# alshai/Big-BWT

Hardware: AMD Instinct MI355X
Metric: input MB/s to .bwt (bit-exact vs ref) (higher is better)
Workload: dtype u8; 1 GPU; BASELINE configs[2]: 64x mutated yeast-shaped FASTA (~0.79 GB), -w 10 -p 100, BWT + -s -e sampled SA; bytes_per_gpu=787308470, w=10, p=100, flags=6, phrases=16409159, words=921010, dict_bytes=79900101, parallelism=1 GPU

## Files before the change

### big-bwt_amd/csrc/api_stages.hip

```cpp
#include "chain.hpp"

using namespace pfp;

namespace pfp {

__global__ void sorted_len1_kernel(uint32_t d, const uint32_t *__restrict__ word_at_rank,
                                   const uint32_t *__restrict__ wlen, uint32_t *__restrict__ len1) {
  uint32_t r = BID * blockDim.x + threadIdx.x;
  if (r == 0) len1[d] = 0;
  if (r < d) len1[r] = wlen[word_at_rank[r]] + 1;
}

template <class A, class B>
__global__ void convert_kernel(const A *__restrict__ in, uint64_t n, B *__restrict__ out) {
  uint64_t i = (uint64_t)BID * blockDim.x + threadIdx.x;
  if (i < n) out[i] = (B)in[i];
}
template <class A, class B>
static void fetch_converted(pfp_ctx *c, const A *d_in, uint64_t n, B *h_out) {
  if constexpr (sizeof(A) == sizeof(B)) {
    d2h(c, (A *)h_out, d_in, n);
    sync(c);
  } else {
    DBuf<B> tmp(c, n);
// ... 308 lines not shown
              pfp_bwt_result *out) {
  if (!c || !dict || !occ || !ilist || !bwlast || !out) return PFP_EINVAL;
  memset(out, 0, sizeof *out);
  PFP_TRY_DEV(c)
  check_args(w, 10, flags);
  PFP_REQUIRE(!flags || bwsai, PFP_EINVAL, "SA output requested but no bwsai given");
  PFP_REQUIRE(dict_size > 1 + (uint64_t)w, PFP_EFORMAT, "invalid dictionary file (pfbwt.cpp:332)");
  PFP_REQUIRE(ilist[0] == 1, PFP_EFORMAT, "ilist[0] != 1 (pfbwt.cpp:377)");
  PFP_REQUIRE(dict[0] == kDollar, PFP_EFORMAT, "dictionary must start with Dollar (pfbwt.cpp:125)");
  Dictionary D; DictIndex ix; DictOrder ord;
  dictionary_from_host(c, dict, dict_size, D, ix);
  PFP_REQUIRE(D.d == n_words, PFP_EFORMAT, "occ entries != dictionary words (pfbwt.cpp:357)");
  uint64_t expect = 0, tot_occ = 0;
  {
    uint64_t s = 0, j = 0;
    for (uint64_t i = 0; i < dict_size; i++)
      if (dict[i] == kEndOfWord) {
        uint64_t len = i - s;
        if (len > (uint64_t)w) expect += (len - (uint64_t)w) * occ[j];
        tot_occ += occ[j];
        j++; s = i + 1;
      }
  }
  PFP_REQUIRE(tot_occ + 1 == n_plus_1, PFP_EFORMAT, "sum(occ)+1 != parse size (pfbwt.cpp:397)");
  D.wocc.alloc(c, D.d);
  h2d(c, D.wocc.p, occ, D.d);
  if (c->debug) validate_index(c, D, ix);
  const WordView wv = word_view(D, ix);
  const SlotPayloadSrc pay{wv, D.wocc.p, w};
  ord.wide = use_wide_index(c, D.dsize);
  with_width(ord.wide, [&](auto tag) {
    using I = decltype(tag);
    auto &so = ord.get<I>();
    sort_dict_suffixes<I>(c, D.bytes.p, D.dsize, wv, so, (flags & PFP_FLAG_SA) ? nullptr : &pay);
    if (c->debug) validate_suffix_order<I>(c, D.bytes.p, so, true, "dict SA");
    compute_lexrank<I>(c, D, so, ix);
  });
  if (c->debug) validate_lexrank(c, D, ix);
  DBuf<uint32_t> occ_lex(c, D.d);
  occ_in_lex_order(c, (uint32_t)D.d, ix.lexrank.p, D.wocc.p, occ_lex.p, nullptr);
  ParseBWT pb;
  pb.P = n_plus_1 - 1;
  pb.ilist.alloc(c, n_plus_1); pb.bwlast.alloc(c, n_plus_1);
  h2d(c, pb.ilist.p, ilist, n_plus_1); h2d(c, pb.bwlast.p, bwlast, n_plus_1);
  if (flags) {
    DBuf<uint8_t> packed(c, n_plus_1 * 5);
    h2d(c, packed.p, bwsai, n_plus_1 * 5);
    pb.bwsai.alloc(c, n_plus_1);
    unpack5_dev(c, packed.p, n_plus_1, pb.bwsai.p);
// ... 19 lines not shown
```

### big-bwt_amd/csrc/chain.hip

```cpp
#include "chain.hpp"

using namespace pfp;

namespace pfp {

__global__ void occ_lex_kernel(uint32_t d, const uint32_t *__restrict__ lexrank, const uint32_t *__restrict__ wocc,
                               uint32_t *__restrict__ occ_lex, uint32_t *__restrict__ word_at_rank) {
  uint32_t j = BID * blockDim.x + threadIdx.x;
  if (j >= d) return;
  uint32_t r = lexrank[j];
  occ_lex[r] = wocc[j];
  if (word_at_rank) word_at_rank[r] = j;
}
__global__ void parse_sym_kernel(uint64_t P, const uint32_t *__restrict__ pid, const uint32_t *__restrict__ lexrank,
                                 uint32_t *__restrict__ sym) {
  uint64_t k = (uint64_t)BID * blockDim.x + threadIdx.x;
  if (k < P) sym[k] = lexrank[pid[k]] + 1;
}
__global__ __launch_bounds__(256) void dict_permute_kernel(uint32_t d, const uint32_t *__restrict__ word_at_rank,
                                                           const uint64_t *__restrict__ woff,
                                                           const uint32_t *__restrict__ wlen,
                                                           const uint8_t *__restrict__ src,
                                                           const uint64_t *__restrict__ doff, uint8_t *__restrict__ dst) {
  uint64_t t = (uint64_t)BID * 256 + threadIdx.x;
// ... 34 lines not shown
    if (c->debug) validate_dictionary(c, ch.D, w);
    build_dict_index(c, ch.D, ch.ix);
    if (c->debug) validate_index(c, ch.D, ch.ix);
    ch.tx.buf.release();
    ch.ends.release();
  }
  {
    PhaseTimer t(c, &st.ms_sa_dict);
    const WordView wv = word_view(ch.D, ch.ix);
    const SlotPayloadSrc pay{wv, ch.D.wocc.p, w};
    ch.ord.wide = prefer_wide_index(c, ch.D.dsize);
    with_width(ch.ord.wide, [&](auto tag) {
      using I = decltype(tag);
      auto &so = ch.ord.get<I>();
      so.rep_hint = (double)ch.n_used / (double)std::max<uint64_t>(ch.D.dsize, 1);
      sort_dict_suffixes<I>(c, ch.D.bytes.p, ch.D.dsize, wv, so, dense_sa ? nullptr : &pay);
      if (c->debug) validate_suffix_order<I>(c, ch.D.bytes.p, so, true, "dict SA");
      compute_lexrank<I>(c, ch.D, so, ch.ix);
      if (!c->debug) { so.rank.release(); so.tab.release(); }
    });
    if (c->debug) validate_lexrank(c, ch.D, ch.ix);
    const uint32_t d = (uint32_t)ch.D.d;
    ch.occ_lex.alloc(c, d); ch.word_at_rank.alloc(c, d);
    occ_in_lex_order(c, d, ch.ix.lexrank.p, ch.D.wocc.p, ch.occ_lex.p, ch.word_at_rank.p);
    ch.sym.alloc(c, ch.D.P);
    hipLaunchKernelGGL(parse_sym_kernel, gdim(cdiv(ch.D.P, TB)), gdim(TB), 0, c->stream, ch.D.P, ch.D.pid.p,
                       ch.ix.lexrank.p, ch.sym.p);
    PFP_HIP(hipGetLastError());
  }
  st.n = ch.n_used; st.n_phrases = ch.D.P; st.n_words = ch.D.d; st.dict_size = ch.D.dsize;
  st.sa_rounds_dict = ch.ord.rounds(); st.hash_reseeds = ch.D.reseeds; st.index_bits = ch.ord.wide ? 64 : 32;
// ... 234 lines not shown
```

### big-bwt_amd/csrc/common.hpp

```cpp
#pragma once
#include <hip/hip_runtime.h>
#include <cstdint>
#include <cstdio>
#include <cstring>
#include <stdexcept>
#include <string>
#include <vector>
#include <chrono>
#include <map>
#include <thread>
#include "../../include/pfpgpu.h"

struct K1Scratch; struct DistState;
namespace pfp {
struct StagedText;

constexpr uint8_t kDollar = 2, kEndOfWord = 1, kEndOfDict = 0;
constexpr uint32_t kPrime = 1999999973u;

struct Error : std::runtime_error {
  int code;
  Error(int c, const std::string &m) : std::runtime_error(m), code(c) {}
};

// ... 77 lines not shown
      free_list[bi] = free_list.back(); free_list.pop_back();
      for (auto &b : all) if (b.p == p) { b.file = file; b.line = line; b.req = bytes; break; }
      note_peak();
      return p;
    }
    void *p = nullptr;
    hipError_t e = hipMalloc(&p, bytes);
    driver_allocs++;
    if (e != hipSuccess) {
      (void)hipGetLastError();
      trim();
      trims++;
      e = hipMalloc(&p, bytes);
    }
    if (e != hipSuccess) { *err = e; (void)hipGetLastError(); return nullptr; }
    all.push_back({p, bytes, p, file, line, bytes}); total_bytes += bytes;
    live_bytes += bytes; note_peak();
    return p;
  }
  void put(void *p) {
    for (size_t i = 0; i < all.size(); i++)
      if (all[i].p == p) {
        live_bytes -= all[i].req;
        if (debug) { put_debug(i); return; }
        free_list.push_back(all[i]);
        return;
      }
  }
  void *get_debug(size_t bytes, hipError_t *err, const char *file, int line) {
    void *base = nullptr;
// ... 192 lines not shown
```

### big-bwt_amd/csrc/kernels.hpp

```cpp
#pragma once
#include "common.hpp"
#include "wordview.hpp"

namespace pfp {

struct StagedText {
  static constexpr size_t kFront = 64, kBack = 128;
  DBuf<uint8_t> buf;
  uint64_t n = 0;
  int w = 0;
  const uint8_t *tbase() const { return buf.p + kFront; }
  const uint8_t *tprime() const { return buf.p + kFront - 1; }
  void stage(pfp_ctx *c, const void *src, bool src_on_device, uint64_t n_, int w_);
  void stage_fd(pfp_ctx *c, int fd, uint64_t file_off, uint64_t n_, int w_);
  void restage_tail(pfp_ctx *c, uint64_t new_n, int w_) const;
};

struct KRParams {
  static constexpr uint32_t kMaxExtra = 32;
  uint32_t negpw, pinv, pshift, plimit;
  float fdens = 1.0f;
  uint32_t fthr_nom = 0, fauto = 0;
  uint32_t fast = 0, fseed = 0, fthr = 0;
  uint32_t nextra;
// ... 89 lines not shown
  uint64_t n_refined = 0;
};
using SuffixOrder = SuffixOrderT<uint32_t>;
using SuffixOrder64 = SuffixOrderT<uint64_t>;
struct SlotPayloadSrc { WordView wv; const uint32_t *wocc; int w; };
template <class I>
struct RankViewT {
  const I *rank; const uint64_t *skeys; const I *tab; const uint32_t *lut; const uint8_t *bytes;
  uint64_t N; int kbits, shift; uint32_t T; I finbit; uint64_t keymask;
  const I *wordrank;
};
template <class I> RankViewT<I> rank_view(const SuffixOrderT<I> &so);
template <class I> void gather_ranks(pfp_ctx *c, const SuffixOrderT<I> &so, const uint64_t *d_pos, uint64_t count, I *d_out);
template <class I>
void sort_dict_suffixes(pfp_ctx *c, const uint8_t *bytes, uint64_t N, const WordView &wv, SuffixOrderT<I> &out,
                        const SlotPayloadSrc *pay = nullptr);
template <class I>
void sort_dict_suffixes_range(pfp_ctx *c, const uint8_t *bytes, uint64_t N, const WordView &wv, uint32_t part,
                              uint32_t parts, SuffixOrderT<I> &out, const SlotPayloadSrc *pay = nullptr,
                              const SlotPayloadSrc *count = nullptr);
template <class I>
void gather_slots_range(pfp_ctx *c, const SuffixOrderT<I> &so, const WordView &wv, uint64_t count, uint64_t *d_out);
void sort_int_suffixes_range(pfp_ctx *c, const uint32_t *sym, uint64_t N, uint32_t max_sym, const uint32_t *occ, uint32_t n_sym,
                             uint32_t part, uint32_t parts, SuffixOrder &out);
void sort_int_suffixes(pfp_ctx *c, const uint32_t *sym, uint64_t N, SuffixOrder &out, uint32_t max_sym = 0xFFFFFFFFu,
                       const uint32_t *occ = nullptr, uint32_t n_sym = 0);
template <class I> void sort_byte_suffixes(pfp_ctx *c, const uint8_t *bytes, uint64_t N, SuffixOrderT<I> &out);

struct DictIndex {
  DBuf<uint32_t> blk_word;
  DBuf<uint64_t> wend;
// ... 239 lines not shown
```

### big-bwt_amd/csrc/merge.hip

```cpp
#include "kernels.hpp"
#include "prims.hpp"
#include "devutil.hpp"
#include <algorithm>
#include <cstdlib>

namespace pfp {

static constexpr int TB = 256;
constexpr int kOffTileLog = 11;


template <class I> struct alignas(16) Idx8 { I v[8]; };
template <class I>
__global__ __launch_bounds__(256) void slot_payload_kernel(uint64_t N, const I *__restrict__ sa,
                                                           const uint64_t *__restrict__ skeys,
                                                           const uint8_t *__restrict__ refined, const uint8_t *__restrict__ b,
                                                           WordView wv,
                                                           const uint32_t *__restrict__ wocc, uint32_t d, int w,
                                                           uint32_t *__restrict__ cnt, uint8_t *__restrict__ pc) {
  if ((uint64_t)BID * 2048 >= N) return;
  uint64_t t0 = ((uint64_t)BID * 256 + threadIdx.x) * 8;
  uint32_t c8[8], p8[8];
  const int nk = t0 >= N ? 0 : ((N - t0) >= 8 ? 8 : (int)(N - t0));
  uint64_t rf = 0;
// ... 1375 lines not shown
    sync(c);
    for (uint32_t q = 0; q < nbig; q++) hg.es[q + 1] = hg.es[q] + hb[q].E;
    hg.estart.alloc(c, nbig + 1);
    PFP_HIP(hipMemcpyAsync(hg.estart.p, hg.es.data(), (nbig + 1) * 8, hipMemcpyHostToDevice, c->stream));
    sync(c);
  }

  void queued_groups(int pass) {
    const MergeArgsT<I> ap = with_pass(pass);
    const std::vector<uint64_t> &es = hg.es;
    if (hg.nmid) {
      KScope ks(c, "pfp::hard_sort_kernel", (uint64_t)hg.nmid * (kHardSortMin + 1) * (sa_mode ? 21 : 5));
      hipLaunchKernelGGL(hard_sort_kernel<I>, gdim(c->n_cu * 4), gdim(256), 0, c->stream, ap, hg.mid.p, hg.nmid);
      PFP_HIP(hipGetLastError());
    }
    for (uint32_t q0 = 0; q0 < hg.nbig;) {
      uint32_t q1 = q0 + 1;
      while (q1 < hg.nbig && es[q1 + 1] - es[q0] <= sw.big_budget) q1++;
      const uint64_t cnt = es[q1] - es[q0];
      if (cnt > sw.big_budget) {
        const int nb = (int)std::min<uint64_t>(cdiv64(cnt, 256), (uint64_t)c->n_cu * 32);
        KScope ks(c, "pfp::hard_big_kernel", cnt * (sa_mode ? 21 : 5));
        hipLaunchKernelGGL(hard_big_kernel<I>, gdim(nb), gdim(256), 0, c->stream, ap, hg.big.p + q0, q1 - q0, hg.estart.p + q0, cnt);
      } else {
        DBuf<uint64_t> bk(c, cnt), bka(c, cnt), bv(c, cnt), bva(c, cnt);
        { KScope ks(c, "pfp::big_keys_kernel", cnt * 28);
          hipLaunchKernelGGL(big_keys_kernel<I>, gdim(cdiv(cnt, 256)), gdim(256), 0, c->stream, ap, hg.big.p, q0, q1, hg.estart.p, cnt, bk.p, bv.p); }
        { SortTag tag("large hard groups"); sort_pairs_db<uint64_t, uint64_t>(c, bk, bka, bv, bva, cnt, 0, 32 + bits_for(q1 - q0)); }
        { KScope ks(c, "pfp::big_place_kernel", cnt * (sa_mode ? 34 : 18));
          hipLaunchKernelGGL(big_place_kernel<I>, gdim(cdiv(cnt, 256)), gdim(256), 0, c->stream, ap, hg.big.p, q0, hg.estart.p, cnt, bk.p, bv.p); }
      }
      PFP_HIP(hipGetLastError());
      q0 = q1;
    }
  }

  void mark_run_boundaries() {
    const uint64_t cnt_slice = a.out_hi > a.out_lo ? a.out_hi - a.out_lo : 0;
    const uint64_t nw = cdiv64(cnt_slice, 64);
    out.bmap.alloc(c, nw + 1); out.bpre.alloc(c, nw + 1);
// ... 129 lines not shown
```

### big-bwt_amd/csrc/sufsort.hip

```cpp
#include "kernels.hpp"
#include "prims.hpp"
#include "devutil.hpp"
#include <algorithm>
#include <cmath>
#include <optional>
#include <vector>
#include <cstdio>
#include <cstdlib>

namespace pfp {

enum : int { MODE_DICT = 0, MODE_PLAIN = 1 };

struct SufGeom {
  int mode; uint64_t N; WordView wv;
  const uint32_t *sym = nullptr;
  const uint32_t *dist = nullptr;
};
__device__ __forceinline__ uint64_t suf_len(const SufGeom &g, uint64_t i) {
  if (g.mode == MODE_DICT) return slen_of(g.wv, i) + 1;
  return g.N - i;
}

struct KeyCode {
// ... 113 lines not shown
    if ((L.skeys[mid] & L.keymask) < k) lo = mid + 1; else hi = mid;
  }
  return lo;
}

__device__ __forceinline__ uint32_t slot_record(const uint8_t *__restrict__ b, uint64_t i, uint32_t wd, const SlotPayloadSrc &P) {
  if (!(wd < P.wv.d && P.wv.wend[wd] - i > (uint64_t)P.w)) return 0u;
  const uint32_t pc = (i == 0) ? kEndOfWord : b[i - 1];
  const uint32_t occ = P.wocc[wd];
  return pc | ((occ < 255u ? occ : 255u) << 8);
}
constexpr int kKeyPos = 224;
struct KeyStreamLds { uint32_t off[257]; uint32_t bs[200]; uint32_t wsum[4]; unsigned long long tmask[4]; uint32_t wbase; };
__device__ __forceinline__ uint64_t block_stream_key(KeyStreamLds &L, const uint8_t *__restrict__ s, uint64_t N,
                                                     const KeyCode &kp, uint64_t B0, const WordView *view = nullptr,
                                                     uint32_t *word_out = nullptr) {
  const int t = threadIdx.x, lane = t & 63, wv = t >> 6;
  const uint64_t pos = B0 + t;
  if (t < 200) L.bs[t] = 0;
  const uint32_t c = pos < N ? s[pos] : 0u;
  const uint32_t e = kp.lut[c];
  const uint32_t l = e & 63u, cd = e >> 6;
  uint32_t inc = l;
  for (int o = 1; o < 64; o <<= 1) { const uint32_t v = __shfl_up(inc, o, 64); if (lane >= o) inc += v; }
  if (lane == 63) L.wsum[wv] = inc;
  const unsigned long long tmine = __ballot(c <= (uint32_t)kEndOfWord);
  if (lane == 0) L.tmask[wv] = tmine;
  if (word_out && t == 0) L.wbase = B0 < N ? word_of(*view, B0) : 0u;
  __syncthreads();
  if (word_out) {
    uint32_t before = (uint32_t)__popcll(tmine & ((1ull << lane) - 1ull));
    for (int q = 0; q < wv; q++) before += (uint32_t)__popcll(L.tmask[q]);
    *word_out = L.wbase + before;
  }
  uint32_t base = 0;
  for (int q = 0; q < wv; q++) base += L.wsum[q];
  const uint32_t p = base + inc - l;
  L.off[t] = p;
  if (t == 255) L.off[256] = p + l;
  {
    const uint32_t w = p >> 5, o = p & 31u;
    if (o + l <= 32) atomicOr(&L.bs[w], cd << (32 - o - l));
    else {
      const uint32_t r = o + l - 32;
      atomicOr(&L.bs[w], cd >> r);
      atomicOr(&L.bs[w + 1], (cd & ((1u << r) - 1u)) << (32 - r));
    }
  }
  __syncthreads();
  if (t >= kKeyPos || pos >= N) return 0;
  uint32_t toterm = 33u;
  {
    const unsigned long long m0 = tmine >> lane;
    if (m0) toterm = (uint32_t)__builtin_ctzll(m0) + 1u;
    else if (wv < 3) { const unsigned long long m1 = L.tmask[wv + 1]; if (m1) toterm = (uint32_t)(64 - lane) + (uint32_t)__builtin_ctzll(m1) + 1u; }
    if (toterm > 33u) toterm = 33u;
  }
  const uint32_t nch = toterm < 32u ? toterm : 32u;
  const uint32_t avail = L.off[t + nch] - p;
  const uint32_t kb = (uint32_t)kp.kbits;
  const uint32_t take = avail < kb ? avail : kb;
  const uint32_t w = p >> 5, sh = p & 31u;
  const uint64_t hi = ((uint64_t)L.bs[w] << 32) | L.bs[w + 1];
  uint64_t x = hi << sh;
  if (sh) x |= (uint64_t)(L.bs[w + 2] >> (32 - sh));
  uint64_t k = x >> (64 - kb);
  if (take < kb) k &= ~((1ull << (kb - take)) - 1ull);
  const uint32_t term = (toterm <= 32u && L.off[t + toterm] - p <= kb) ? 1u : 0u;
  return (k << 1) | term;
}
template <class I>
__global__ __launch_bounds__(256) void init_keys_packed_kernel(const uint8_t *__restrict__ s, uint64_t N, KeyCode kp,
                                                               SlotPayloadSrc P, int paybits, uint64_t *__restrict__ key,
                                                               I *__restrict__ val, int idx_bits) {
  __shared__ KeyStreamLds L;
  const uint64_t B0 = (uint64_t)BID * kKeyPos;
  uint32_t wd = 0;
  uint64_t k = paybits ? block_stream_key(L, s, N, kp, B0, &P.wv, &wd) : block_stream_key(L, s, N, kp, B0);
  const uint64_t pos = B0 + threadIdx.x;
  if (threadIdx.x >= kKeyPos || pos >= N) return;
  if (idx_bits) { key[pos] = (k << idx_bits) | pos; return; }
  if (paybits) k |= (uint64_t)slot_record(s, pos, wd, P) << 48;
  key[pos] = k; val[pos] = (I)pos;
}
template <class I>
__global__ void split_keys_kernel(const uint64_t *__restrict__ comb, uint64_t n, int idx_bits, uint64_t *__restrict__ key,
                                  I *__restrict__ val) {
  const uint64_t a = (uint64_t)BID * blockDim.x + threadIdx.x;
  if (a >= n) return;
  const uint64_t x = comb[a];
  key[a] = x >> idx_bits;
  val[a] = (I)(x & ((1ull << idx_bits) - 1ull));
}
__global__ void check_keys_kernel(const uint8_t *__restrict__ s, uint64_t N, KeyCode kp, const uint64_t *__restrict__ key,
                                  uint64_t keymask, unsigned long long *__restrict__ bad, int idx_bits) {
  uint64_t i = (uint64_t)BID * blockDim.x + threadIdx.x;
  if (i >= N) return;
  if (((key[i] >> idx_bits) & keymask) != packed_key_at(s, i, kp.kbits, kp.lut)) atomicAdd(bad, 1ull);
}
template <class I>
__global__ void init_keys_bytes_kernel(const uint8_t *__restrict__ s, uint64_t N, uint64_t *__restrict__ key,
                                       I *__restrict__ val) {
  uint64_t i = (uint64_t)BID * blockDim.x + threadIdx.x;
  if (i >= N) return;
  key[i] = __builtin_bswap64(ld8u(s + i));
  val[i] = (I)i;
}
__global__ void init_keys_int_kernel(const uint32_t *__restrict__ s, uint64_t N, uint64_t *__restrict__ key,
                                     uint32_t *__restrict__ val) {
  uint64_t i = (uint64_t)BID * blockDim.x + threadIdx.x;
  if (i >= N) return;
  uint64_t a = s[i], b = (i + 1 < N) ? s[i + 1] : 0;
  key[i] = (a << 32) | b; val[i] = (uint32_t)i;
// ... 551 lines not shown
  uint32_t pivot_cap = []() { const char *e = getenv("PFP_PIVOT_CAP"); uint32_t v = e ? (uint32_t)atoll(e) : 512u; return v > kPivCapMax ? kPivCapMax : v; }();
};
static const SorterSwitches kSwitch;

template <class I>
RankViewT<I> rank_view(const SuffixOrderT<I> &so) {
  return RankViewT<I>{so.rank.p, so.skeys.p, so.tab.p, so.lut.p, so.bytes, so.N, so.kbits, so.shift, so.T, so.finbit, so.keymask, so.wordrank.p};
}
template RankViewT<uint32_t> rank_view(const SuffixOrderT<uint32_t> &);
template RankViewT<uint64_t> rank_view(const SuffixOrderT<uint64_t> &);

struct DoublingOpts {
  int key_bits = 64;
  bool dict = false;
  std::optional<uint64_t> list_len;
  int idx_bits = 0;
};

enum class Round {
  FirstDict,
  FirstPlain,
  DictPivotGlobal,
  DictPivotGrouped,
  ParsePivot,
  DoublingGlobal,
  DoublingGrouped,
};

template <class I>
struct Rounds {
  using K = typename IdxTraits<I>::DKey;
  static constexpr bool kWide = sizeof(I) == 8;
  static constexpr int TB = 256;

  pfp_ctx *const c;
  const SufGeom g;
  SuffixOrderT<I> &out;
  const DoublingOpts o;
  const uint64_t NP, N;
  const bool lazy;
  const bool range_mode;
  const int nb;
  bool lazy_active = false, late_rank = false;
  I *rank_p = nullptr, *wordrank_p = nullptr;

  Round kind;
  uint64_t m, h, m2 = 0, ngrp = 0;
  uint32_t piv_cap = kSwitch.pivot_cap;
  bool pivot_ok = true;
  bool ipiv_ok = true;
  bool small_failed = false;
  bool finisher_ok = true;
  bool rank_alloc = false;
  bool lazy_pending = false;
  bool ranks_stale = false;
// ... 5 lines not shown
  DBuf<uint64_t> keyo;
  DBuf<I> valo;
  DBuf<uint8_t> hd, keep;
  DBuf<I> aslot, aslot2, hv, newhead, act_i, act_grp;
  uint64_t list_cap = 0;
  DBuf<uint32_t> tile_keep, tile_heads;
  DBuf<I> tile_off, tile_hoff;
  DBuf<uint8_t> keep0, veto;
  DBuf<uint32_t> wstart_bits;
  DBuf<uint8_t> gs, bigf;
  DBuf<uint32_t> k32, k32o, segb, sege, nseg_d, ovf_d;
  DBuf<uint64_t> nsel_d;
  DBuf<K> dkey, dkeyo;

  Rounds(pfp_ctx *c_, const SufGeom &g_, DBuf<uint64_t> &key_, DBuf<I> &val_, uint64_t h0, SuffixOrderT<I> &out_, const DoublingOpts &o_)
      : c(c_), g(g_), out(out_), o(o_), NP(g_.N), N(o_.list_len.value_or(g_.N)), lazy(o_.dict), range_mode(o_.list_len.has_value()),
        nb(bits_for(N)), kind(o_.dict ? Round::FirstDict : Round::FirstPlain), m(N), h(h0), key(key_), val(val_) {}

  static uint64_t blocks(uint64_t n) { return cdiv(n, TB); }

  void first_round_sort() {
    keyo.alloc(c, N); valo.alloc(c, N);
    SortTag first_tag(g.mode == MODE_DICT ? "dictionary, first round" : "parse, first round");
    if (o.idx_bits) {
      if (kSwitch.lib_sort) sort_keys_db(c, key, keyo, N, o.idx_bits, o.idx_bits + o.key_bits);
      else msd_sort_keys_db(c, key, keyo, N, o.idx_bits, o.idx_bits + o.key_bits);
      KScope ks(c, "pfp::split_keys_kernel", N * (16 + sizeof(I)));
      hipLaunchKernelGGL(split_keys_kernel<I>, gdim(blocks(N)), gdim(TB), 0, c->stream, key.p, N, o.idx_bits, keyo.p, valo.p);
    } else {
      if (kSwitch.lib_sort) sort_pairs_db(c, key, keyo, val, valo, N, 0, o.key_bits);
      else msd_sort_pairs_db<I>(c, key, keyo, val, valo, N, 0, o.key_bits);
// ... 359 lines not shown
      if (kind != Round::DoublingGrouped) {
        { KScope ks(c, "pfp::build_keys_kernel", m * (4 + 4 + 4 + 12));
          hipLaunchKernelGGL(build_keys_kernel<I>, gdim(blocks(m)), gdim(TB), 0, c->stream, g, m, h, act_i.p, act_grp.p, L, nb, key.p, val.p); }
        sort_device_wide(keybits);
      }
    }
    h *= 2;
    out.rounds++;
  }

  bool next_round() {
    if (dict_pivot_wanted()) { dict_pivot_round(); return true; }
    if constexpr (!kWide) {
      if (parse_pivot_wanted() && parse_pivot_round()) return true;
    }
    if (range_mode) { out.complete = false; return false; }
    prepare_ranks_for_doubling();
    doubling_round();
    return true;
  }
};

template <class I>
static void doubling(pfp_ctx *c, SufGeom g, DBuf<uint64_t> &key, DBuf<I> &val, uint64_t h0, SuffixOrderT<I> &out, const DoublingOpts &o) {
  Rounds<I> r(c, g, key, val, h0, out, o);
  out.N = r.N; out.NP = r.NP; out.range = r.range_mode; out.complete = true;
  out.rounds = 0;
  if (r.N == 0) { out.sa.alloc(c, 1); out.grp.alloc(c, 8); out.rank.alloc(c, 1); return; }
  r.first_round_sort();
  SortTag later_tag(g.mode == MODE_DICT ? "dictionary, later rounds" : "parse, later rounds");
  r.start_rounds();
// ... 17 lines not shown
    const I r = L.wordrank[a];
    if (r != IdxTraits<I>::kNone) { out[a] = r & ~L.finbit; return; }
  }
  out[a] = rank_at(L, pos[a], settled);
}
template <class I>
void gather_ranks(pfp_ctx *c, const SuffixOrderT<I> &so, const uint64_t *d_pos, uint64_t count, I *d_out) {
  if (!count) return;
  hipLaunchKernelGGL(gather_ranks_kernel<I>, gdim(cdiv(count, 256)), gdim(256), 0, c->stream, rank_view(so), count, d_pos, d_out);
  PFP_HIP(hipGetLastError());
}
template void gather_ranks<uint32_t>(pfp_ctx *, const SuffixOrderT<uint32_t> &, const uint64_t *, uint64_t, uint32_t *);
template void gather_ranks<uint64_t>(pfp_ctx *, const SuffixOrderT<uint64_t> &, const uint64_t *, uint64_t, uint64_t *);


static KeyCode dict_key_code(pfp_ctx *c, const uint8_t *bytes, uint64_t N, double rep_hint = 0) {
  DBuf<unsigned long long> hist(c, 256);
  hist.zero();
  hipLaunchKernelGGL(byte_histogram_kernel, gdim(std::min<uint64_t>(cdiv64(N, 4096), (uint64_t)c->n_cu * 8)), gdim(256), 0,
                     c->stream, bytes, N, hist.p);
  std::vector<uint64_t> hh(256);
  PFP_HIP(hipMemcpyAsync(hh.data(), hist.p, 2048, hipMemcpyDeviceToHost, c->stream));
  sync(c);
  return make_key_code(hh.data(), rep_hint);
}

template <class I>
static int keysonly_bits(uint64_t N, double rep_hint, KeyCode &kc) {
  const int keysonly_env = []() { const char *e = getenv("PFP_KEYSONLY"); return e ? atoi(e) : -1; }();
  if (!(sizeof(I) == 4 && N >= 2 && (keysonly_env == 1 || (keysonly_env != 0 && rep_hint >= 2.0 && N >= (1u << 20))))) return 0;
  const int ib = bits_for(N - 1);
  int width = 64 - ib;
  if (width > 3 * kKeysDigitBits && width % kKeysDigitBits <= 2) width -= width % kKeysDigitBits;
  if (!(width - 1 >= 35 || keysonly_env == 1)) return 0;
  if (kc.kbits > width - 1) { kc.kbits = std::max(8, width - 1); kc.hmin = std::max(1, std::min(32, kc.kbits / kc.maxlen)); }
  return ib;
}

template <class I>
static void require_dict_size(uint64_t N) {
  PFP_REQUIRE(N >= 1 && (sizeof(I) == 8 ? N < (1ull << 40) : N < 0xFFFFFFF0ull), PFP_ELIMIT,
              sizeof(I) == 8 ? "dictionary of 2^40 bytes or more" : "dictionary too large for 32-bit suffix indices");
}
static uint64_t dict_keymask(const KeyCode &kc) { return kc.kbits + 1 >= 64 ? ~0ull : ((1ull << (kc.kbits + 1)) - 1); }

template <class I>
static void dict_rounds(pfp_ctx *c, const SufGeom &g, const uint8_t *bytes, const KeyCode &kc, int idx_bits, std::optional<uint64_t> list_len,
                        DBuf<uint64_t> &key, DBuf<I> &val, SuffixOrderT<I> &out) {
  out.keymask = dict_keymask(kc);
  out.lut.alloc(c, 256);
  PFP_HIP(hipMemcpyAsync(out.lut.p, kc.lut, 1024, hipMemcpyHostToDevice, c->stream));
  sync(c);
  out.bytes = bytes; out.kbits = kc.kbits;
  DoublingOpts o;
  o.key_bits = kc.kbits + 1, o.dict = true, o.list_len = list_len, o.idx_bits = idx_bits;
  doubling<I>(c, g, key, val, (uint64_t)kc.hmin, out, o);
}

template <class I>
void sort_dict_suffixes(pfp_ctx *c, const uint8_t *bytes, uint64_t N, const WordView &wv, SuffixOrderT<I> &out,
                        const SlotPayloadSrc *pay) {
  require_dict_size<I>(N);
  SufGeom g{MODE_DICT, N, wv};
  KeyCode kc = dict_key_code(c, bytes, N, out.rep_hint);
  const int idx_bits = keysonly_bits<I>(N, out.rep_hint, kc);
  DBuf<uint64_t> key(c, N);
  DBuf<I> val;
  if (!idx_bits) val.alloc(c, N);
  out.paybits = (pay && !idx_bits && kc.kbits + 1 <= 48) ? 16 : 0;
  { KScope ks(c, "pfp::init_keys_packed_kernel", N * (9 + (idx_bits ? 0 : sizeof(I)) + (out.paybits ? 9 : 0)));
    hipLaunchKernelGGL(init_keys_packed_kernel<I>, gdim((unsigned)cdiv64(N, kKeyPos)), gdim(256), 0, c->stream, bytes, N, kc,
                       pay ? *pay : SlotPayloadSrc{}, out.paybits, key.p, val.p, idx_bits); }
  if (c->debug) {
    DBuf<unsigned long long> bad(c, 1);
    bad.zero();
    hipLaunchKernelGGL(check_keys_kernel, gdim(cdiv(N, 256)), gdim(256), 0, c->stream, bytes, N, kc, key.p, dict_keymask(kc), bad.p, idx_bits);
    PFP_HIP(hipMemcpyAsync(c->h_scalars, bad.p, 8, hipMemcpyDeviceToHost, c->stream));
    sync(c);
    PFP_REQUIRE(c->h_scalars[0] == 0, PFP_EHIP, "bit-stream keys differ from packed_key_at at " + std::to_string(c->h_scalars[0]) + " positions");
  }
  dict_rounds<I>(c, g, bytes, kc, idx_bits, std::nullopt, key, val, out);
}
template void sort_dict_suffixes<uint32_t>(pfp_ctx *, const uint8_t *, uint64_t, const WordView &, SuffixOrderT<uint32_t> &, const SlotPayloadSrc *);
template void sort_dict_suffixes<uint64_t>(pfp_ctx *, const uint8_t *, uint64_t, const WordView &, SuffixOrderT<uint64_t> &, const SlotPayloadSrc *);


template <class I>
void sort_byte_suffixes(pfp_ctx *c, const uint8_t *bytes, uint64_t N, SuffixOrderT<I> &out) {
  PFP_REQUIRE(N >= 1 && (sizeof(I) == 8 ? N < (1ull << 40) : N < 0xFFFFFFF0ull), PFP_ELIMIT, "text too large for the suffix index width");
  SufGeom g{MODE_PLAIN, N, WordView{}};
  DBuf<uint64_t> key(c, N);
  DBuf<I> val(c, N);
  { KScope ks(c, "pfp::init_keys_bytes_kernel", N * (16 + sizeof(I)));
    hipLaunchKernelGGL(init_keys_bytes_kernel<I>, gdim(cdiv(N, 256)), gdim(256), 0, c->stream, bytes, N, key.p, val.p); }
  doubling<I>(c, g, key, val, 8, out, DoublingOpts{});
}
template void sort_byte_suffixes<uint32_t>(pfp_ctx *, const uint8_t *, uint64_t, SuffixOrderT<uint32_t> &);
template void sort_byte_suffixes<uint64_t>(pfp_ctx *, const uint8_t *, uint64_t, SuffixOrderT<uint64_t> &);

// ... 279 lines not shown
                                                 SuffixOrderT<uint64_t> &, const SlotPayloadSrc *, const SlotPayloadSrc *);

template <class I>
__global__ void word_slots_range_kernel(uint64_t N, const I *__restrict__ sa, WordView wv, uint64_t slot_base, uint64_t *__restrict__ out) {
  const uint64_t t = (uint64_t)BID * blockDim.x + threadIdx.x;
  if (t >= N) return;
  const uint64_t i = sa[t];
  if (i != 0 && wv.bytes[i - 1] != kEndOfWord) return;
  const uint32_t wd = word_of(wv, i);
  if (wd < wv.d) out[wd] = slot_base + t + 1;
}
template <class I>
void gather_slots_range(pfp_ctx *c, const SuffixOrderT<I> &so, const WordView &wv, uint64_t count, uint64_t *d_out) {
  if (!count) return;
  PFP_HIP(hipMemsetAsync(d_out, 0, count * 8, c->stream));
  if (so.N) hipLaunchKernelGGL(word_slots_range_kernel<I>, gdim(cdiv(so.N, 256)), gdim(256), 0, c->stream, so.N, so.sa.p, wv, so.slot_base, d_out);
  PFP_HIP(hipGetLastError());
}
template void gather_slots_range<uint32_t>(pfp_ctx *, const SuffixOrderT<uint32_t> &, const WordView &, uint64_t, uint64_t *);
template void gather_slots_range<uint64_t>(pfp_ctx *, const SuffixOrderT<uint64_t> &, const WordView &, uint64_t, uint64_t *);

__global__ void sample_u64_kernel(const uint64_t *__restrict__ key, uint64_t stride, uint32_t ns, uint64_t *__restrict__ out, uint32_t *__restrict__ idx) {
  uint32_t j = BID * blockDim.x + threadIdx.x;
  if (j < ns) { out[j] = key[(uint64_t)j * stride]; idx[j] = j; }
}
__global__ __launch_bounds__(256) void range_flags_u64_kernel(const uint64_t *__restrict__ key, uint64_t N, uint64_t klo, uint64_t khi, int khi_open,
                                                              uint8_t *__restrict__ flag, unsigned long long *__restrict__ tile_below) {
  __shared__ unsigned long long ws[4];
  const uint64_t i = (uint64_t)BID * 256 + threadIdx.x;
  unsigned long long lt = 0;
// ... 53 lines not shown
```

### big-bwt_amd/csrc/validate.hip

```cpp
#include "kernels.hpp"
#include <algorithm>

namespace pfp {

template <class T>
static std::vector<T> fetch(pfp_ctx *c, const T *d, size_t n) {
  std::vector<T> h(n);
  if (n) PFP_HIP(hipMemcpyAsync(h.data(), d, n * sizeof(T), hipMemcpyDeviceToHost, c->stream));
  sync(c);
  return h;
}
#define VFAIL(msg) throw Error(PFP_EFORMAT, std::string("PFP_DEBUG validation failed: ") + msg)

void validate_scan(pfp_ctx *c, const DBuf<uint64_t> &ends, uint64_t n_ends, uint64_t n, int w) {
  auto e = fetch(c, ends.p, n_ends);
  for (uint64_t k = 0; k < n_ends; k++) {
    if (e[k] >= n || e[k] + 1 < (uint64_t)w) VFAIL("scan: end out of range at " + std::to_string(k));
    if (k && e[k] <= e[k - 1]) VFAIL("scan: ends not increasing at " + std::to_string(k));
  }
}

void validate_dictionary(pfp_ctx *c, const Dictionary &D, int w) {
  auto pid = fetch(c, D.pid.p, D.P);
  auto wlen = fetch(c, D.wlen.p, D.d);
// ... 40 lines not shown
  }
  if (wd != D.d || we[D.d] != D.dsize - 1) VFAIL("index: word count");
}

static int cmp_suffix(const std::vector<uint8_t> &b, uint64_t x, uint64_t y) {
  for (;;) {
    uint8_t cx = b[x], cy = b[y];
    if (cx != cy) return cx < cy ? -1 : 1;
    if (cx <= kEndOfWord) return 0;
    x++; y++;
  }
}

template <class I>
void validate_suffix_order(pfp_ctx *c, const uint8_t *bytes, SuffixOrderT<I> &so, bool dict_mode, const char *what) {
  const uint64_t N = so.N;
  auto sa = fetch(c, so.sa.p, N);
  std::vector<I> rk(N);
  {
    std::vector<uint64_t> pos(N);
    for (uint64_t i = 0; i < N; i++) pos[i] = i;
    DBuf<uint64_t> dpos(c, N);
    DBuf<I> dr(c, N);
    h2d(c, dpos.p, pos.data(), N);
    gather_ranks<I>(c, so, dpos.p, N, dr.p);
    rk = fetch(c, dr.p, N);
  }
  auto gr = fetch(c, so.grp.p, N);
  std::vector<uint8_t> seen(N, 0);
  for (uint64_t t = 0; t < N; t++) {
    if (sa[t] >= N || seen[sa[t]]) VFAIL(std::string(what) + ": sa is not a permutation at slot " + std::to_string(t));
    seen[sa[t]] = 1;
    if (rk[sa[t]] > t) VFAIL(std::string(what) + ": rank above slot");
    if (rk[sa[t]] != gr[t]) VFAIL(std::string(what) + ": rank lookup differs from the slot's group head at slot " + std::to_string(t));
  }
  if (dict_mode && N < (64u << 20)) {
    auto b = fetch(c, bytes, N);
    for (uint64_t t = 1; t < N; t++) {
      int cmp = cmp_suffix(b, sa[t - 1], sa[t]);
      bool same = rk[sa[t - 1]] == rk[sa[t]];
      if (cmp > 0) VFAIL(std::string(what) + ": suffixes out of order at slot " + std::to_string(t));
      if ((cmp == 0) != same) VFAIL(std::string(what) + ": rank equality != string equality at slot " + std::to_string(t));
      if (cmp == 0 && sa[t - 1] > sa[t]) VFAIL(std::string(what) + ": equal suffixes not in position order");
    }
  }
}

template void validate_suffix_order<uint32_t>(pfp_ctx *, const uint8_t *, SuffixOrderT<uint32_t> &, bool, const char *);
template void validate_suffix_order<uint64_t>(pfp_ctx *, const uint8_t *, SuffixOrderT<uint64_t> &, bool, const char *);

void validate_int_sa(pfp_ctx *c, const uint32_t *sym, const SuffixOrder &so) {
  const uint64_t N = so.N;
  auto sa = fetch(c, so.sa.p, N);
  auto s = fetch(c, sym, N);
  std::vector<uint8_t> seen(N, 0);
  for (uint64_t t = 0; t < N; t++) {
    if (sa[t] >= N || seen[sa[t]]) VFAIL("parse SA is not a permutation");
    seen[sa[t]] = 1;
// ... 29 lines not shown
```

Before: 28090 MB/s.

## Skip sorting dictionary suffixes shorter than the window in dict SA

Dictionary suffixes of at most w bytes never contribute to the BWT, so the key-init kernel now compacts only the suffixes longer than w into the sort list and doubling runs in list mode over that smaller set. Word bases are computed from the 64-byte block word table plus a ballot popcount. If the short list still needs a doubling round, or the dictionary has a short word or stray low byte, it falls back to sorting every position. It also reuses the big-group sort buffers across iterations instead of reallocating them each time. This adds extra checks and a possible full re-sort as the cost.

```diff
diff --git a/big-bwt_amd/csrc/api_stages.hip b/big-bwt_amd/csrc/api_stages.hip
--- a/big-bwt_amd/csrc/api_stages.hip
+++ b/big-bwt_amd/csrc/api_stages.hip
@@ -346,13 +346,16 @@
   uint64_t expect = 0, tot_occ = 0;
   {
     uint64_t s = 0, j = 0;
-    for (uint64_t i = 0; i < dict_size; i++)
+    for (uint64_t i = 0; i < dict_size; i++) {
+      PFP_REQUIRE(dict[i] >= kDollar || dict[i] == kEndOfWord || i + 1 == dict_size, PFP_EFORMAT,
+                  "invalid dictionary file: byte 0x00 inside a word at offset " + std::to_string(i));
       if (dict[i] == kEndOfWord) {
         uint64_t len = i - s;
         if (len > (uint64_t)w) expect += (len - (uint64_t)w) * occ[j];
         tot_occ += occ[j];
         j++; s = i + 1;
       }
+    }
   }
   PFP_REQUIRE(tot_occ + 1 == n_plus_1, PFP_EFORMAT, "sum(occ)+1 != parse size (pfbwt.cpp:397)");
   D.wocc.alloc(c, D.d);
@@ -364,7 +367,7 @@
   with_width(ord.wide, [&](auto tag) {
     using I = decltype(tag);
     auto &so = ord.get<I>();
-    sort_dict_suffixes<I>(c, D.bytes.p, D.dsize, wv, so, (flags & PFP_FLAG_SA) ? nullptr : &pay);
+    sort_dict_suffixes<I>(c, D.bytes.p, D.dsize, wv, so, (flags & PFP_FLAG_SA) ? nullptr : &pay, w);
     if (c->debug) validate_suffix_order<I>(c, D.bytes.p, so, true, "dict SA");
     compute_lexrank<I>(c, D, so, ix);
   });
diff --git a/big-bwt_amd/csrc/chain.hip b/big-bwt_amd/csrc/chain.hip
--- a/big-bwt_amd/csrc/chain.hip
+++ b/big-bwt_amd/csrc/chain.hip
@@ -72,7 +72,7 @@
       using I = decltype(tag);
       auto &so = ch.ord.get<I>();
       so.rep_hint = (double)ch.n_used / (double)std::max<uint64_t>(ch.D.dsize, 1);
-      sort_dict_suffixes<I>(c, ch.D.bytes.p, ch.D.dsize, wv, so, dense_sa ? nullptr : &pay);
+      sort_dict_suffixes<I>(c, ch.D.bytes.p, ch.D.dsize, wv, so, dense_sa ? nullptr : &pay, w);
       if (c->debug) validate_suffix_order<I>(c, ch.D.bytes.p, so, true, "dict SA");
       compute_lexrank<I>(c, ch.D, so, ch.ix);
       if (!c->debug) { so.rank.release(); so.tab.release(); }
diff --git a/big-bwt_amd/csrc/common.hpp b/big-bwt_amd/csrc/common.hpp
--- a/big-bwt_amd/csrc/common.hpp
+++ b/big-bwt_amd/csrc/common.hpp
@@ -115,6 +115,7 @@
       e = hipMalloc(&p, bytes);
     }
     if (e != hipSuccess) { *err = e; (void)hipGetLastError(); return nullptr; }
+    if (trace) fprintf(stderr, "[pfp] pool: driver allocation %llu of %zu bytes for %s:%d\n", (unsigned long long)driver_allocs, bytes, file, line);
     all.push_back({p, bytes, p, file, line, bytes}); total_bytes += bytes;
     live_bytes += bytes; note_peak();
     return p;
diff --git a/big-bwt_amd/csrc/kernels.hpp b/big-bwt_amd/csrc/kernels.hpp
--- a/big-bwt_amd/csrc/kernels.hpp
+++ b/big-bwt_amd/csrc/kernels.hpp
@@ -127,7 +127,7 @@
 template <class I> void gather_ranks(pfp_ctx *c, const SuffixOrderT<I> &so, const uint64_t *d_pos, uint64_t count, I *d_out);
 template <class I>
 void sort_dict_suffixes(pfp_ctx *c, const uint8_t *bytes, uint64_t N, const WordView &wv, SuffixOrderT<I> &out,
-                        const SlotPayloadSrc *pay = nullptr);
+                        const SlotPayloadSrc *pay = nullptr, int min_len = 0);
 template <class I>
 void sort_dict_suffixes_range(pfp_ctx *c, const uint8_t *bytes, uint64_t N, const WordView &wv, uint32_t part,
                               uint32_t parts, SuffixOrderT<I> &out, const SlotPayloadSrc *pay = nullptr,
diff --git a/big-bwt_amd/csrc/merge.hip b/big-bwt_amd/csrc/merge.hip
--- a/big-bwt_amd/csrc/merge.hip
+++ b/big-bwt_amd/csrc/merge.hip
@@ -1413,6 +1413,8 @@
       hipLaunchKernelGGL(hard_sort_kernel<I>, gdim(c->n_cu * 4), gdim(256), 0, c->stream, ap, hg.mid.p, hg.nmid);
       PFP_HIP(hipGetLastError());
     }
+    const uint64_t max_cnt = std::min<uint64_t>(sw.big_budget, es[hg.nbig]);
+    DBuf<uint64_t> bk, bka, bv, bva;
     for (uint32_t q0 = 0; q0 < hg.nbig;) {
       uint32_t q1 = q0 + 1;
       while (q1 < hg.nbig && es[q1 + 1] - es[q0] <= sw.big_budget) q1++;
@@ -1422,7 +1424,7 @@
         KScope ks(c, "pfp::hard_big_kernel", cnt * (sa_mode ? 21 : 5));
         hipLaunchKernelGGL(hard_big_kernel<I>, gdim(nb), gdim(256), 0, c->stream, ap, hg.big.p + q0, q1 - q0, hg.estart.p + q0, cnt);
       } else {
-        DBuf<uint64_t> bk(c, cnt), bka(c, cnt), bv(c, cnt), bva(c, cnt);
+        if (!bk.p) { bk.alloc(c, max_cnt); bka.alloc(c, max_cnt); bv.alloc(c, max_cnt); bva.alloc(c, max_cnt); }
         { KScope ks(c, "pfp::big_keys_kernel", cnt * 28);
           hipLaunchKernelGGL(big_keys_kernel<I>, gdim(cdiv(cnt, 256)), gdim(256), 0, c->stream, ap, hg.big.p, q0, q1, hg.estart.p, cnt, bk.p, bv.p); }
         { SortTag tag("large hard groups"); sort_pairs_db<uint64_t, uint64_t>(c, bk, bka, bv, bva, cnt, 0, 32 + bits_for(q1 - q0)); }
diff --git a/big-bwt_amd/csrc/sufsort.hip b/big-bwt_amd/csrc/sufsort.hip
--- a/big-bwt_amd/csrc/sufsort.hip
+++ b/big-bwt_amd/csrc/sufsort.hip
@@ -151,7 +151,7 @@
 struct KeyStreamLds { uint32_t off[257]; uint32_t bs[200]; uint32_t wsum[4]; unsigned long long tmask[4]; uint32_t wbase; };
 __device__ __forceinline__ uint64_t block_stream_key(KeyStreamLds &L, const uint8_t *__restrict__ s, uint64_t N,
                                                      const KeyCode &kp, uint64_t B0, const WordView *view = nullptr,
-                                                     uint32_t *word_out = nullptr) {
+                                                     uint32_t *word_out = nullptr, uint32_t *toterm_out = nullptr) {
   const int t = threadIdx.x, lane = t & 63, wv = t >> 6;
   const uint64_t pos = B0 + t;
   if (t < 200) L.bs[t] = 0;
@@ -163,7 +163,14 @@
   if (lane == 63) L.wsum[wv] = inc;
   const unsigned long long tmine = __ballot(c <= (uint32_t)kEndOfWord);
   if (lane == 0) L.tmask[wv] = tmine;
-  if (word_out && t == 0) L.wbase = B0 < N ? word_of(*view, B0) : 0u;
+  if (word_out) {
+    const unsigned long long t1 = __ballot(c == (uint32_t)kEndOfWord);
+    if (t == 0) {
+      const uint64_t line = (B0 >> 6) + 1;
+      const uint32_t upto = (uint32_t)(line * 64 - B0);
+      L.wbase = B0 < N ? view->blk_word[line] - (uint32_t)__popcll(upto >= 64 ? t1 : (t1 & ((1ull << upto) - 1ull))) : 0u;
+    }
+  }
   __syncthreads();
   if (word_out) {
     uint32_t before = (uint32_t)__popcll(tmine & ((1ull << lane) - 1ull));
@@ -193,6 +200,7 @@
     else if (wv < 3) { const unsigned long long m1 = L.tmask[wv + 1]; if (m1) toterm = (uint32_t)(64 - lane) + (uint32_t)__builtin_ctzll(m1) + 1u; }
     if (toterm > 33u) toterm = 33u;
   }
+  if (toterm_out) *toterm_out = toterm;
   const uint32_t nch = toterm < 32u ? toterm : 32u;
   const uint32_t avail = L.off[t + nch] - p;
   const uint32_t kb = (uint32_t)kp.kbits;
@@ -206,19 +214,36 @@
   const uint32_t term = (toterm <= 32u && L.off[t + toterm] - p <= kb) ? 1u : 0u;
   return (k << 1) | term;
 }
+__device__ __forceinline__ bool suffix_kept(const WordView &v, uint32_t wd, uint64_t pos, int min_len) {
+  return wd < v.d && v.wend[wd] - pos > (uint64_t)min_len;
+}
+__global__ void short_words_kernel(WordView view, int min_len, unsigned long long *__restrict__ found) {
+  const uint32_t j = BID * blockDim.x + threadIdx.x;
+  if (j >= view.d) return;
+  const uint64_t start = j ? view.wend[j - 1] + 1 : 0;
+  if (view.wend[j] - start <= (uint64_t)min_len) *found = 1ull;
+}
 template <class I>
 __global__ __launch_bounds__(256) void init_keys_packed_kernel(const uint8_t *__restrict__ s, uint64_t N, KeyCode kp,
                                                                SlotPayloadSrc P, int paybits, uint64_t *__restrict__ key,
-                                                               I *__restrict__ val, int idx_bits) {
+                                                               I *__restrict__ val, int idx_bits, WordView view, int min_len,
+                                                               uint64_t listed ) {
   __shared__ KeyStreamLds L;
   const uint64_t B0 = (uint64_t)BID * kKeyPos;
-  uint32_t wd = 0;
-  uint64_t k = paybits ? block_stream_key(L, s, N, kp, B0, &P.wv, &wd) : block_stream_key(L, s, N, kp, B0);
+  uint32_t wd = 0, toterm = 0;
+  uint64_t k = (paybits || listed) ? block_stream_key(L, s, N, kp, B0, &view, &wd, &toterm) : block_stream_key(L, s, N, kp, B0);
   const uint64_t pos = B0 + threadIdx.x;
   if (threadIdx.x >= kKeyPos || pos >= N) return;
-  if (idx_bits) { key[pos] = (k << idx_bits) | pos; return; }
+  uint64_t at = pos;
+  if (listed) {
+    const bool keep = min_len < 32 ? toterm > (uint32_t)min_len + 1u : suffix_kept(view, wd, pos, min_len);
+    if (!keep) return;
+    at = pos - ((uint64_t)min_len + 1) * wd;
+    if (at >= listed) return;
+  }
+  if (idx_bits) { key[at] = (k << idx_bits) | pos; return; }
   if (paybits) k |= (uint64_t)slot_record(s, pos, wd, P) << 48;
-  key[pos] = k; val[pos] = (I)pos;
+  key[at] = k; val[at] = (I)pos;
 }
 template <class I>
 __global__ void split_keys_kernel(const uint64_t *__restrict__ comb, uint64_t n, int idx_bits, uint64_t *__restrict__ key,
@@ -229,11 +254,23 @@
   key[a] = x >> idx_bits;
   val[a] = (I)(x & ((1ull << idx_bits) - 1ull));
 }
-__global__ void check_keys_kernel(const uint8_t *__restrict__ s, uint64_t N, KeyCode kp, const uint64_t *__restrict__ key,
-                                  uint64_t keymask, unsigned long long *__restrict__ bad, int idx_bits) {
-  uint64_t i = (uint64_t)BID * blockDim.x + threadIdx.x;
-  if (i >= N) return;
-  if (((key[i] >> idx_bits) & keymask) != packed_key_at(s, i, kp.kbits, kp.lut)) atomicAdd(bad, 1ull);
+template <class I>
+__global__ void check_keys_kernel(const uint8_t *__restrict__ s, uint64_t n, KeyCode kp, const uint64_t *__restrict__ key,
+                                  const I *__restrict__ val, uint64_t keymask, unsigned long long *__restrict__ bad, int idx_bits,
+                                  int listed, WordView view, int min_len) {
+  uint64_t a = (uint64_t)BID * blockDim.x + threadIdx.x;
+  if (a >= n) return;
+  uint64_t i = a;
+  if (listed) {
+    auto pos_at = [&](uint64_t q) { return idx_bits ? (key[q] & ((1ull << idx_bits) - 1ull)) : (uint64_t)val[q]; };
+    i = pos_at(a);
+    const uint64_t from = a ? pos_at(a - 1) + 1 : 0;
+    bool ok = i < view.NP && from <= i && suffix_kept(view, word_of(view, i), i, min_len);
+    for (uint64_t j = from; ok && j < i; j++) ok = !suffix_kept(view, word_of(view, j), j, min_len);
+    if (ok && a + 1 == n) for (uint64_t j = i + 1; ok && j < view.NP; j++) ok = !suffix_kept(view, word_of(view, j), j, min_len);
+    if (!ok) { atomicAdd(bad, 1ull); return; }
+  }
+  if (((key[a] >> idx_bits) & keymask) != packed_key_at(s, i, kp.kbits, kp.lut)) atomicAdd(bad, 1ull);
 }
 template <class I>
 __global__ void init_keys_bytes_kernel(const uint8_t *__restrict__ s, uint64_t N, uint64_t *__restrict__ key,
@@ -815,6 +852,7 @@
   int key_bits = 64;
   bool dict = false;
   std::optional<uint64_t> list_len;
+  bool whole_list = false;
   int idx_bits = 0;
 };
 
@@ -840,6 +878,7 @@
   const DoublingOpts o;
   const uint64_t NP, N;
   const bool lazy;
+  const bool list_mode;
   const bool range_mode;
   const int nb;
   bool lazy_active = false, late_rank = false;
@@ -875,7 +914,8 @@
   DBuf<K> dkey, dkeyo;
 
   Rounds(pfp_ctx *c_, const SufGeom &g_, DBuf<uint64_t> &key_, DBuf<I> &val_, uint64_t h0, SuffixOrderT<I> &out_, const DoublingOpts &o_)
-      : c(c_), g(g_), out(out_), o(o_), NP(g_.N), N(o_.list_len.value_or(g_.N)), lazy(o_.dict), range_mode(o_.list_len.has_value()),
+      : c(c_), g(g_), out(out_), o(o_), NP(g_.N), N(o_.list_len.value_or(g_.N)), lazy(o_.dict), list_mode(o_.list_len.has_value()),
+        range_mode(o_.list_len.has_value() && !o_.whole_list),
         nb(bits_for(N)), kind(o_.dict ? Round::FirstDict : Round::FirstPlain), m(N), h(h0), key(key_), val(val_) {}
 
   static uint64_t blocks(uint64_t n) { return cdiv(n, TB); }
@@ -1265,7 +1305,7 @@
     if constexpr (!kWide) {
       if (parse_pivot_wanted() && parse_pivot_round()) return true;
     }
-    if (range_mode) { out.complete = false; return false; }
+    if (list_mode) { out.complete = false; return false; }
     prepare_ranks_for_doubling();
     doubling_round();
     return true;
@@ -1313,7 +1353,7 @@
 template void gather_ranks<uint64_t>(pfp_ctx *, const SuffixOrderT<uint64_t> &, const uint64_t *, uint64_t, uint64_t *);
 
 
-static KeyCode dict_key_code(pfp_ctx *c, const uint8_t *bytes, uint64_t N, double rep_hint = 0) {
+static KeyCode dict_key_code(pfp_ctx *c, const uint8_t *bytes, uint64_t N, double rep_hint = 0, uint64_t *low_counts = nullptr) {
   DBuf<unsigned long long> hist(c, 256);
   hist.zero();
   hipLaunchKernelGGL(byte_histogram_kernel, gdim(std::min<uint64_t>(cdiv64(N, 4096), (uint64_t)c->n_cu * 8)), gdim(256), 0,
@@ -1321,6 +1361,7 @@
   std::vector<uint64_t> hh(256);
   PFP_HIP(hipMemcpyAsync(hh.data(), hist.p, 2048, hipMemcpyDeviceToHost, c->stream));
   sync(c);
+  if (low_counts) { low_counts[0] = hh[0]; low_counts[1] = hh[1]; }
   return make_key_code(hh.data(), rep_hint);
 }
 
@@ -1345,43 +1386,71 @@
 
 template <class I>
 static void dict_rounds(pfp_ctx *c, const SufGeom &g, const uint8_t *bytes, const KeyCode &kc, int idx_bits, std::optional<uint64_t> list_len,
-                        DBuf<uint64_t> &key, DBuf<I> &val, SuffixOrderT<I> &out) {
+                        DBuf<uint64_t> &key, DBuf<I> &val, SuffixOrderT<I> &out, bool whole_list = false) {
   out.keymask = dict_keymask(kc);
   out.lut.alloc(c, 256);
   PFP_HIP(hipMemcpyAsync(out.lut.p, kc.lut, 1024, hipMemcpyHostToDevice, c->stream));
   sync(c);
   out.bytes = bytes; out.kbits = kc.kbits;
   DoublingOpts o;
-  o.key_bits = kc.kbits + 1, o.dict = true, o.list_len = list_len, o.idx_bits = idx_bits;
+  o.key_bits = kc.kbits + 1, o.dict = true, o.list_len = list_len, o.whole_list = whole_list, o.idx_bits = idx_bits;
   doubling<I>(c, g, key, val, (uint64_t)kc.hmin, out, o);
 }
 
+static bool drop_short_enabled() { const char *e = getenv("PFP_DROP_SHORT"); return !e || atoi(e) != 0; }
+
 template <class I>
 void sort_dict_suffixes(pfp_ctx *c, const uint8_t *bytes, uint64_t N, const WordView &wv, SuffixOrderT<I> &out,
-                        const SlotPayloadSrc *pay) {
+                        const SlotPayloadSrc *pay, int min_len) {
   require_dict_size<I>(N);
   SufGeom g{MODE_DICT, N, wv};
-  KeyCode kc = dict_key_code(c, bytes, N, out.rep_hint);
+  const uint64_t ntile = cdiv64(N, kKeyPos);
+  const uint64_t dropped = (uint64_t)wv.d * ((uint64_t)min_len + 1) + 1;
+  bool listed = min_len > 0 && wv.d >= 1 && dropped < N && drop_short_enabled();
+  unsigned long long *const short_found = reinterpret_cast<unsigned long long *>(c->h_scalars + 3);
+  if (listed) {
+    *short_found = 0;
+    KScope ks(c, "pfp::short_words_kernel", (uint64_t)wv.d * 8);
+    hipLaunchKernelGGL(short_words_kernel, gdim(cdiv((uint64_t)wv.d, 256)), gdim(256), 0, c->stream, wv, min_len, short_found);
+  }
+  uint64_t low_counts[2] = {0, 0};
+  KeyCode kc = dict_key_code(c, bytes, N, out.rep_hint, low_counts);
+  if (listed && (*short_found != 0 || low_counts[0] != 1 || low_counts[1] != (uint64_t)wv.d)) {
+    listed = false;
+    if (kSwitch.trace_rounds)
+      fprintf(stderr, "[pfp] dictionary with a word of at most %d bytes or a stray byte below 2: every position is sorted\n", min_len);
+  }
+  const uint64_t n = listed ? N - dropped : N;
   const int idx_bits = keysonly_bits<I>(N, out.rep_hint, kc);
-  DBuf<uint64_t> key(c, N);
+  DBuf<uint64_t> key(c, n);
   DBuf<I> val;
-  if (!idx_bits) val.alloc(c, N);
+  if (!idx_bits) val.alloc(c, n);
   out.paybits = (pay && !idx_bits && kc.kbits + 1 <= 48) ? 16 : 0;
-  { KScope ks(c, "pfp::init_keys_packed_kernel", N * (9 + (idx_bits ? 0 : sizeof(I)) + (out.paybits ? 9 : 0)));
-    hipLaunchKernelGGL(init_keys_packed_kernel<I>, gdim((unsigned)cdiv64(N, kKeyPos)), gdim(256), 0, c->stream, bytes, N, kc,
-                       pay ? *pay : SlotPayloadSrc{}, out.paybits, key.p, val.p, idx_bits); }
+  { KScope ks(c, "pfp::init_keys_packed_kernel", N + n * (8 + (idx_bits ? 0 : sizeof(I)) + (out.paybits ? 9 : 0)));
+    hipLaunchKernelGGL(init_keys_packed_kernel<I>, gdim((unsigned)ntile), gdim(256), 0, c->stream, bytes, N, kc,
+                       pay ? *pay : SlotPayloadSrc{}, out.paybits, key.p, val.p, idx_bits, wv, min_len, listed ? n : (uint64_t)0); }
   if (c->debug) {
     DBuf<unsigned long long> bad(c, 1);
     bad.zero();
-    hipLaunchKernelGGL(check_keys_kernel, gdim(cdiv(N, 256)), gdim(256), 0, c->stream, bytes, N, kc, key.p, dict_keymask(kc), bad.p, idx_bits);
+    hipLaunchKernelGGL(check_keys_kernel<I>, gdim(cdiv(n, 256)), gdim(256), 0, c->stream, bytes, n, kc, key.p, val.p, dict_keymask(kc), bad.p,
+                       idx_bits, listed ? 1 : 0, wv, min_len);
     PFP_HIP(hipMemcpyAsync(c->h_scalars, bad.p, 8, hipMemcpyDeviceToHost, c->stream));
     sync(c);
     PFP_REQUIRE(c->h_scalars[0] == 0, PFP_EHIP, "bit-stream keys differ from packed_key_at at " + std::to_string(c->h_scalars[0]) + " positions");
   }
-  dict_rounds<I>(c, g, bytes, kc, idx_bits, std::nullopt, key, val, out);
-}
-template void sort_dict_suffixes<uint32_t>(pfp_ctx *, const uint8_t *, uint64_t, const WordView &, SuffixOrderT<uint32_t> &, const SlotPayloadSrc *);
-template void sort_dict_suffixes<uint64_t>(pfp_ctx *, const uint8_t *, uint64_t, const WordView &, SuffixOrderT<uint64_t> &, const SlotPayloadSrc *);
+  if (!listed) { dict_rounds<I>(c, g, bytes, kc, idx_bits, std::nullopt, key, val, out); return; }
+  dict_rounds<I>(c, g, bytes, kc, idx_bits, n, key, val, out, true);
+  if (out.complete) return;
+  if (kSwitch.trace_rounds) fprintf(stderr, "[pfp] the sort of the %llu suffixes longer than %d bytes needs a doubling round: every position is sorted\n",
+                                    (unsigned long long)n, min_len);
+  key.release(); val.release();
+  const double rep_hint = out.rep_hint;
+  out = SuffixOrderT<I>{};
+  out.rep_hint = rep_hint;
+  sort_dict_suffixes<I>(c, bytes, N, wv, out, pay, 0);
+}
+template void sort_dict_suffixes<uint32_t>(pfp_ctx *, const uint8_t *, uint64_t, const WordView &, SuffixOrderT<uint32_t> &, const SlotPayloadSrc *, int);
+template void sort_dict_suffixes<uint64_t>(pfp_ctx *, const uint8_t *, uint64_t, const WordView &, SuffixOrderT<uint64_t> &, const SlotPayloadSrc *, int);
 
 
 template <class I>
@@ -1691,6 +1760,7 @@
 void gather_slots_range(pfp_ctx *c, const SuffixOrderT<I> &so, const WordView &wv, uint64_t count, uint64_t *d_out) {
   if (!count) return;
   PFP_HIP(hipMemsetAsync(d_out, 0, count * 8, c->stream));
+  KScope ks(c, "pfp::word_slots_range_kernel", so.N * (sizeof(I) + 1) + count * 8);
   if (so.N) hipLaunchKernelGGL(word_slots_range_kernel<I>, gdim(cdiv(so.N, 256)), gdim(256), 0, c->stream, so.N, so.sa.p, wv, so.slot_base, d_out);
   PFP_HIP(hipGetLastError());
 }
diff --git a/big-bwt_amd/csrc/validate.hip b/big-bwt_amd/csrc/validate.hip
--- a/big-bwt_amd/csrc/validate.hip
+++ b/big-bwt_amd/csrc/validate.hip
@@ -78,12 +78,16 @@
 
 template <class I>
 void validate_suffix_order(pfp_ctx *c, const uint8_t *bytes, SuffixOrderT<I> &so, bool dict_mode, const char *what) {
-  const uint64_t N = so.N;
+  const uint64_t N = so.N, NP = so.NP ? so.NP : so.N;
+  if (N > NP) VFAIL(std::string(what) + ": more slots than positions");
   auto sa = fetch(c, so.sa.p, N);
   std::vector<I> rk(N);
   {
     std::vector<uint64_t> pos(N);
-    for (uint64_t i = 0; i < N; i++) pos[i] = i;
+    for (uint64_t t = 0; t < N; t++) {
+      if (sa[t] >= NP) VFAIL(std::string(what) + ": sa is not a permutation at slot " + std::to_string(t));
+      pos[t] = sa[t];
+    }
     DBuf<uint64_t> dpos(c, N);
     DBuf<I> dr(c, N);
     h2d(c, dpos.p, pos.data(), N);
@@ -91,21 +95,31 @@
     rk = fetch(c, dr.p, N);
   }
   auto gr = fetch(c, so.grp.p, N);
-  std::vector<uint8_t> seen(N, 0);
+  std::vector<uint8_t> seen(NP, 0);
   for (uint64_t t = 0; t < N; t++) {
-    if (sa[t] >= N || seen[sa[t]]) VFAIL(std::string(what) + ": sa is not a permutation at slot " + std::to_string(t));
+    if (seen[sa[t]]) VFAIL(std::string(what) + ": sa is not a permutation at slot " + std::to_string(t));
     seen[sa[t]] = 1;
-    if (rk[sa[t]] > t) VFAIL(std::string(what) + ": rank above slot");
-    if (rk[sa[t]] != gr[t]) VFAIL(std::string(what) + ": rank lookup differs from the slot's group head at slot " + std::to_string(t));
+    if (rk[t] > t) VFAIL(std::string(what) + ": rank above slot");
+    if (rk[t] != gr[t]) VFAIL(std::string(what) + ": rank lookup differs from the slot's group head at slot " + std::to_string(t));
   }
-  if (dict_mode && N < (64u << 20)) {
-    auto b = fetch(c, bytes, N);
+  if (dict_mode && NP < (64u << 20)) {
+    auto b = fetch(c, bytes, NP);
     for (uint64_t t = 1; t < N; t++) {
       int cmp = cmp_suffix(b, sa[t - 1], sa[t]);
-      bool same = rk[sa[t - 1]] == rk[sa[t]];
+      bool same = rk[t - 1] == rk[t];
       if (cmp > 0) VFAIL(std::string(what) + ": suffixes out of order at slot " + std::to_string(t));
       if ((cmp == 0) != same) VFAIL(std::string(what) + ": rank equality != string equality at slot " + std::to_string(t));
       if (cmp == 0 && sa[t - 1] > sa[t]) VFAIL(std::string(what) + ": equal suffixes not in position order");
+    }
+    if (N < NP) {
+      auto len_at = [&](uint64_t i) { uint64_t l = 0; while (b[i + l] > kEndOfWord) l++; return l; };
+      uint64_t min_kept = ~0ull;
+      for (uint64_t t = 0; t < N; t++) min_kept = std::min(min_kept, len_at(sa[t]));
+      for (uint64_t i = 0; i < NP; i++) {
+        if (seen[i]) continue;
+        if (len_at(i) >= min_kept) VFAIL(std::string(what) + ": a suffix as long as a sorted one was left out at position " + std::to_string(i));
+        if (i + 1 < NP && (i == 0 || b[i - 1] == kEndOfWord)) VFAIL(std::string(what) + ": a whole word was left out at position " + std::to_string(i));
+      }
     }
   }
 }
```

After: 28630 MB/s, median of 6. +1.9%, better.
